# sqeazy/sqeazy

Hardware: AMD Instinct MI355X
Metric: encode GB/s (input voxels) for bitswap1->lz4 uint16 volume (higher is better)
Workload: dtype u16

## Files before the change

sqeazy_amd/csrc/sqy_kernels.hip:

```cpp
#include <hip/hip_runtime.h>
#include <atomic>
#include <mutex>
#include <stdint.h>
#include <cstring>
#include <type_traits>

#include "sqy_kernels.h"
#include "sqy_pipeline.hpp"
#include "sqy_quantiser_lut.hpp"
#include "sqy_batch_view.hpp"
#include "sqy_batch_window.hpp"

namespace sqy {

struct __attribute__((packed)) pk_u16 { uint16_t v; };
struct __attribute__((packed)) pk_u32 { uint32_t v; };
struct __attribute__((packed)) pk_u64 { uint64_t v; };
struct __attribute__((packed)) pk_u128 { uint32_t x, y, z, w; };

__device__ __forceinline__ uint32_t ld_u32(const uint8_t* p) { return reinterpret_cast<const pk_u32*>(p)->v; }
__device__ __forceinline__ uint64_t ld_u64(const uint8_t* p) { return reinterpret_cast<const pk_u64*>(p)->v; }
__device__ __forceinline__ uint4 ld_u128(const uint8_t* p)
{
    const pk_u128 t = *reinterpret_cast<const pk_u128*>(p);
// ... 633 lines not shown
    {
        const uint16_t* prev = out + (uint64_t)(z0 - 1u) * frame;
#pragma unroll
        for (uint32_t k = 0; k < DDK_ITEMS; ++k) {
            if (!it_on[k]) continue;
            uint16_t* d = img[0] + (size_t)it_i[k] * pitch + 8u;
            if (it_v[k] < vpr) *reinterpret_cast<uint4*>(d + it_v[k] * 8u) = *reinterpret_cast<const uint4*>(prev + (uint64_t)it_y[k] * X + it_v[k] * 8u);
            else d[w] = w < X ? prev[(uint64_t)it_y[k] * X + w] : (uint16_t)0;
        }
    }
    uint4 cin[DDK_ITEMS];
#pragma unroll
    for (uint32_t k = 0; k < DDK_ITEMS; ++k) cin[k] = active(k, 0) ? fetch(k, 0) : make_uint4(0, 0, 0, 0);
    __syncthreads();
    int cur = 0;
    for (uint32_t j = 0; j < nframes; ++j) {
        const uint32_t z = z0 + j;
        uint4 nin[DDK_ITEMS];
#pragma unroll
        for (uint32_t k = 0; k < DDK_ITEMS; ++k) nin[k] = (j + 1u < nframes && active(k, j + 1u)) ? fetch(k, j + 1u) : make_uint4(0, 0, 0, 0);
        uint16_t* dst = out + (uint64_t)z * frame;
        const uint16_t* A = img[cur];
        uint16_t* B = img[cur ^ 1];
        const bool frame_touched = z >= 1u && z < zlim && hx > 0u;
#pragma unroll
        for (uint32_t k = 0; k < DDK_ITEMS; ++k) {
            if (!active(k, j)) continue;
            const uint32_t i = it_i[k], v = it_v[k];
            const int32_t y = it_y[k];
            if (v == vpr) {
                B[(size_t)i * pitch + 8u + w] = (uint16_t)cin[k].x;
                continue;
            }
            const uint32_t x0 = v * 8u;
            const uint4 c = cin[k];
            uint32_t val[8] = {c.x & 0xffffu, c.x >> 16, c.y & 0xffffu, c.y >> 16, c.z & 0xffffu, c.z >> 16, c.w & 0xffffu, c.w >> 16};
            if (frame_touched && y >= 1 && y + 2 <= (int32_t)Y && x0 < 1u + hx) {
                uint32_t colsum[10];
#pragma unroll
                for (int q = 0; q < 10; ++q) colsum[q] = 0;
#pragma unroll
                for (int dy = -1; dy <= 1; ++dy) {
                    const uint16_t* r = A + (size_t)((int32_t)i + dy) * pitch + 8u + x0;
                    const uint4 e = *reinterpret_cast<const uint4*>(r);
                    colsum[0] += r[-1];
                    colsum[1] += e.x & 0xffffu; colsum[2] += e.x >> 16; colsum[3] += e.y & 0xffffu; colsum[4] += e.y >> 16;
                    colsum[5] += e.z & 0xffffu; colsum[6] += e.z >> 16; colsum[7] += e.w & 0xffffu; colsum[8] += e.w >> 16;
                    colsum[9] += r[8];
                }
#pragma unroll
                for (int q = 0; q < 8; ++q) {
                    const uint32_t x = x0 + (uint32_t)q;
                    if (x >= 1u && x < 1u + hx) {
                        const uint32_t sum = (colsum[q] + colsum[q + 1] + colsum[q + 2]) & 0xffffu;
                        val[q] = (val[q] + ((sum * 58255u) >> 19)) & 0xffffu;
                    }
                }
            }
            const uint4 o = make_uint4(val[0] | (val[1] << 16), val[2] | (val[3] << 16), val[4] | (val[5] << 16), val[6] | (val[7] << 16));
            *reinterpret_cast<uint4*>(B + (size_t)i * pitch + 8u + x0) = o;
            if (y >= y0 && y < y0 + (int32_t)DDK_R) *reinterpret_cast<uint4*>(dst + (uint64_t)y * X + x0) = o;
        }
        __syncthreads();
        cur ^= 1;
#pragma unroll
        for (uint32_t k = 0; k < DDK_ITEMS; ++k) cin[k] = nin[k];
    }
}

__global__ __launch_bounds__(DDK_THREADS)
void diff3x3x1_u16_decode_frames_kernel(const uint16_t* __restrict__ in, uint16_t* __restrict__ out, uint32_t Y, uint32_t X, uint32_t hx,
                                        uint32_t zlim, uint32_t w, uint32_t z0, uint32_t nframes)
{
    diff3x3x1_u16_decode_strip(in, out, Y, X, hx, zlim, w, z0, nframes, (int32_t)(blockIdx.x * DDK_R));
}

__device__ __forceinline__ uint32_t batch_job_of(const uint32_t* __restrict__ first, uint32_t njobs, uint32_t block)
{
    uint32_t lo = 0, hi = njobs;
    while (hi - lo > 1u) {
        const uint32_t mid = (lo + hi) >> 1;
        if (first[mid] <= block) lo = mid; else hi = mid;
    }
    return lo;
}

__global__ __launch_bounds__(256)
void diff3x3x1_decode_batch_copy_kernel(const DiffBatchJob* __restrict__ jobs, const uint32_t* __restrict__ first_tile, uint32_t njobs)
{
    const uint32_t j = batch_job_of(first_tile, njobs, blockIdx.x);
    const DiffBatchJob job = jobs[j];
    const uint32_t tile = blockIdx.x - first_tile[j];
    const uint32_t vpr = job.X / 8u, wv = job.w / 8u, zlim = job.X < job.Z ? job.X : job.Z;
    const uint64_t fv = (uint64_t)job.Y * vpr, nvec = (uint64_t)job.Z * fv;
    const uint4* __restrict__ in = static_cast<const uint4*>(job.in);
    uint4* __restrict__ out = static_cast<uint4*>(job.out);
#pragma unroll 4
    for (uint32_t i = 0; i < BSWB_THREAD_VOX / 8u; ++i) {
        const uint64_t v = (uint64_t)tile * (BSWB_TILE_VOX / 8u) + i * 256u + threadIdx.x;
        if (v >= nvec) break;
        const uint32_t z = (uint32_t)(v / fv), xv = (uint32_t)((v - (uint64_t)z * fv) % vpr);
        if (z >= 1u && z < zlim && xv < wv) continue;
        out[v] = in[v];
    }
}

__global__ __launch_bounds__(DDK_THREADS)
void diff3x3x1_decode_batch_kernel(const DiffBatchJob* __restrict__ jobs, const uint32_t* __restrict__ first_strip, uint32_t njobs, uint32_t step)
{
    const uint32_t j = batch_job_of(first_strip, njobs, blockIdx.x);
    const DiffBatchJob job = jobs[j];
    const uint32_t strip = blockIdx.x - first_strip[j];
    const uint32_t zlim = job.X < job.Z ? job.X : job.Z, z0 = 1u + step * DDK_K;
    if (z0 >= zlim) return;
    const uint32_t nframes = zlim - z0 < DDK_K ? zlim - z0 : DDK_K;
    diff3x3x1_u16_decode_strip(static_cast<const uint16_t*>(job.in), static_cast<uint16_t*>(job.out), job.Y, job.X, job.Z - 2u, zlim, job.w, z0, nframes,
                               (int32_t)(strip * DDK_R));
}

constexpr uint32_t LZ4_MFLIMIT = 12, LZ4_LASTLITERALS = 5, LZ4_MINLENGTH = 13, LZ4_MAXD = 65535;

__device__ __forceinline__ uint32_t lz4_hash5(uint64_t seq)
{
    return (uint32_t)(((seq << 24) * 889523592379ULL) >> 52);
}

__device__ __forceinline__ uint32_t lz4_hash5_32(uint32_t lo, uint32_t byte4)
{
    const uint32_t plo = 0x1BBCDCBBu;
    const uint32_t l = lo * plo;
    uint32_t h = __umulhi(lo, plo);
    h += (lo & 0xffu) * 0xCFu + (byte4 & 0xffu) * 0xBBu;
    return ((h << 4) | (l >> 28)) & 0xfffu;
}

#ifdef SQY_EXP_STATS
__device__ unsigned long long* g_exp_buf;
__device__ unsigned long long g_exp_cap;
extern "C" __attribute__((visibility("default"))) int SQYAMD_Exp_Set_Buffer(void* p, unsigned long long cap_records)
{
    unsigned long long* q = static_cast<unsigned long long*>(p);
    if (hipMemcpyToSymbol(HIP_SYMBOL(g_exp_buf), &q, sizeof q) != hipSuccess) return 1;
    return hipMemcpyToSymbol(HIP_SYMBOL(g_exp_cap), &cap_records, sizeof cap_records) != hipSuccess;
}
#define SQY_EXP(...) __VA_ARGS__
#else
#define SQY_EXP(...)
#endif
constexpr uint32_t LZ4_RINGLESS_U = 64u * 15u;
#ifndef SQY_EXP_WIN_LEAN
#define SQY_EXP_WIN_LEAN 8192
#endif
#ifndef SQY_EXP_DG_AHEAD
#define SQY_EXP_DG_AHEAD 8
#endif
constexpr uint32_t LZ4_WIN_LEAN = SQY_EXP_WIN_LEAN, LZ4_WIN_DENSE = 32768, LZ4_FB = 1024, LZ4_AHEAD = 2048, LZ4_MIRROR = 16;

template <uint32_t LZ4_WIN>
struct Lz4WindowT {
    glb_u8* src;
    lds_u8* win;
    uint32_t n;
    uint32_t whi, wlo;
    uint32_t nif;
    uint32_t lane16;
    uint32_t pmin;
    SQY_EXP(unsigned long long x_wait = 0; uint32_t x_nwait = 0;)

    __device__ __forceinline__ void issue()
    {
        const uint32_t b = whi + nif * LZ4_FB;
        if (b + LZ4_FB - wlo > LZ4_WIN) wlo = b + LZ4_FB - LZ4_WIN;
        const uint32_t a = b + lane16;
        if (a + 16u <= n) {
            const uint32_t lds_dst = (uint32_t)(uintptr_t)win + (b & (LZ4_WIN - 1));
            uint32_t keep;
            asm volatile("s_mov_b32 %0, m0\n\ts_mov_b32 m0, %2\n\ts_nop 0\n\tglobal_load_lds_dwordx4 %1, off\n\ts_mov_b32 m0, %0"
                         : "=&s"(keep) : "v"(src + a), "s"(lds_dst) : "memory");
        }
        nif += 1;
    }
    __device__ __forceinline__ void commit()
    {
        SQY_EXP(const unsigned long long x_t0 = __builtin_amdgcn_s_memtime();)
        asm volatile("s_waitcnt vmcnt(0)" ::: "memory");
        SQY_EXP(x_wait += __builtin_amdgcn_s_memtime() - x_t0; x_nwait += 1;)
        wave_lds_sync();
        const uint32_t end = whi + nif * LZ4_FB;
        if (((end - 1u) & ~(LZ4_WIN - 1)) != ((whi - 1u) & ~(LZ4_WIN - 1)) || whi == 0) {
            if (lane16 < 64u) *reinterpret_cast<SQY_LDS uint32_t*>(win + LZ4_WIN + (lane16 >> 2)) = *reinterpret_cast<const SQY_LDS uint32_t*>(win + (lane16 >> 2));
            wave_lds_sync();
        }
        whi = end;
        nif = 0;
    }
    __device__ __forceinline__ void ensure(uint32_t ip)
    {
        if (ip + LZ4_AHEAD <= whi || whi >= n) return;
        if (ip >= whi + (LZ4_WIN - LZ4_FB)) {
            asm volatile("s_waitcnt vmcnt(0)" ::: "memory");
            uint32_t start = ip & ~(LZ4_FB - 1);
            if (start >= pmin + LZ4_FB) start -= LZ4_FB;
            whi = wlo = start;
            nif = 0;
        }
        while (whi + nif * LZ4_FB < ip + LZ4_AHEAD && whi + nif * LZ4_FB < n) issue();
        commit();
        if (whi < n) issue();
    }
    __device__ __forceinline__ uint32_t hi_valid() const { return whi < (n & ~15u) ? whi : (n & ~15u); }
    __device__ __forceinline__ bool inside(uint32_t p, uint32_t len) const { return p >= wlo && p + len <= hi_valid(); }
    __device__ __forceinline__ const lds_u8* at(uint32_t p) const { return win + (p & (LZ4_WIN - 1)); }

    __device__ __forceinline__ uint4 lds128(uint32_t p) const { return lds_ld_u128(at(p)); }
    __device__ __forceinline__ uint32_t lds32(uint32_t p) const { return lds_ld_u32(at(p)); }
    __device__ __forceinline__ uint32_t lds8(uint32_t p) const { return lds_ld_u8(at(p)); }

    __device__ __forceinline__ uint64_t rd64(uint32_t p) const
    {
        uint64_t v;
        if (inside(p, 8)) v = lds_ld_u64(at(p)); else v = glb_ld_u64(src + p);
        return v;
    }
    __device__ __forceinline__ uint32_t rd32(uint32_t p) const
    {
        uint32_t v;
        if (inside(p, 4)) v = lds_ld_u32(at(p)); else v = glb_ld_u32(src + p);
        return v;
    }
    __device__ __forceinline__ uint32_t rd8(uint32_t p) const
    {
        uint32_t v;
        if (inside(p, 1)) v = lds_ld_u8(at(p)); else v = glb_ld_u8(src + p);
        return v;
    }
    __device__ __forceinline__ uint4 rd128(uint32_t p) const
    {
        uint4 v;
        if (inside(p, 16)) v = lds_ld_u128(at(p)); else v = glb_ld_u128(src + p);
        return v;
    }
};

template <class Lz4Window>
__device__ __forceinline__ void wave_copy(uint8_t* __restrict__ d, const Lz4Window& w, uint32_t from, uint32_t len, int lane)
{
    if (len <= 64) {
        if ((uint32_t)lane < len) d[lane] = (uint8_t)w.rd8(from + lane);
        return;
    }
    const uint32_t head = (uint32_t)((16 - (reinterpret_cast<uintptr_t>(d) & 15)) & 15);
    if ((uint32_t)lane < head) d[lane] = (uint8_t)w.rd8(from + lane);
    d += head; from += head; len -= head;
    const uint32_t nvec = len >> 4;
    for (uint32_t i = lane; i < nvec; i += 64) {
        *reinterpret_cast<uint4*>(d + (size_t)i * 16) = w.rd128(from + i * 16);
    }
    const uint32_t done = nvec << 4;
    if ((uint32_t)lane < len - done) d[done + lane] = (uint8_t)w.rd8(from + done + lane);
}

__device__ __forceinline__ uint32_t ffbl(uint32_t v)
{
    uint32_t r;
    asm("v_ffbl_b32 %0, %1" : "=v"(r) : "v"(v));
    return r;
}
__device__ __forceinline__ uint32_t first_nonzero16(uint32_t x0, uint32_t x1, uint32_t x2, uint32_t x3)
{
    const uint32_t t0 = ffbl(x0);
    const uint32_t t1 = ffbl(x1) | 32u;
    const uint32_t t2 = ffbl(x2) | 64u;
    const uint32_t t3 = ffbl(x3) | 96u;
    const uint32_t a = t0 < t1 ? t0 : t1, b = t2 < t3 ? t2 : t3;
    const uint32_t m = a < b ? a : b;
    return (m < 128u ? m : 128u) >> 3;
}
__device__ __forceinline__ uint32_t first_diff16(uint4 x, uint4 y)
{
    const uint32_t t0 = ffbl(x.x ^ y.x);
    const uint32_t t1 = ffbl(x.y ^ y.y) | 32u;
    const uint32_t t2 = ffbl(x.z ^ y.z) | 64u;
    const uint32_t t3 = ffbl(x.w ^ y.w) | 96u;
    const uint32_t a = t0 < t1 ? t0 : t1, b = t2 < t3 ? t2 : t3;
    const uint32_t m = a < b ? a : b;
    return (m < 128u ? m : 128u) >> 3;
}

template <class Lz4Window>
__device__ __forceinline__ uint32_t common16(const Lz4Window& w, uint32_t a, uint32_t b, uint32_t maxlen)
{
    if (a + 16u <= w.n) {
        const uint32_t c = first_diff16(w.rd128(a), w.rd128(b));
        return c < maxlen ? c : maxlen;
    }
    uint32_t c = 0;
    while (c < maxlen && glb_ld_u8(w.src + a + c) == glb_ld_u8(w.src + b + c)) ++c;
    return c;
}

constexpr uint32_t LZ4_OB = 2048;

struct Lz4Out {
    SQY_GLB uint8_t* dst;
    lds_u8* ob;
    uint32_t base;
    int lane;
// ... 93 lines not shown
                    za = (qa.x | qa.y | qa.z | qa.w) == 0u;
                    zb = (qb.x | qb.y | qb.z | qb.w) == 0u;
                }
            }
            x[u] = za ? zero : (v4u)a[pc * 64u + lane];
            y[u] = zb ? zero : (v4u)b[pc * 64u + lane];
        }
        uint32_t d = 0;
#pragma unroll
        for (uint32_t u = 0; u < 4; ++u) d |= (x[u].x ^ y[u].x) | (x[u].y ^ y[u].y) | (x[u].z ^ y[u].z) | (x[u].w ^ y[u].w);
        diff = ballot(d != 0u) != 0ull ? 1u : 0u;
    }
    if (lane == 0) dd.dup_of[k] = diff ? (uint32_t)k : r;
    return diff == 0u;
}

template <bool LINKED> struct Lz4ExtraArgs { typedef Lz4DedupeArgs type; };
template <> struct Lz4ExtraArgs<true> { typedef Lz4SpecArgs type; };
__device__ __forceinline__ uint32_t lz4_linked_tag_shift(uint32_t max_block)
{
    const uint32_t pmax = LZ4_HIST + max_block;
    return 31u - (32u - (uint32_t)__builtin_clz(pmax - 1));
}

template <bool LINKED, bool DENSE, bool ACCEL = false, bool TABLE = false>
__global__ __launch_bounds__(64)
void lz4_chunks_kernel(const uint8_t* __restrict__ in, uint64_t total, uint32_t chunk, uint64_t in_stride,
                       uint8_t* __restrict__ scratch, uint64_t stride, uint32_t* __restrict__ csize,
                       const uint64_t* __restrict__ fmap, uint64_t fbytes,
                       const Lz4Block* __restrict__ blocks, const uint32_t* __restrict__ frame_first, uint32_t max_block,
                       uint32_t* __restrict__ redo_list, const uint32_t* __restrict__ dup_of, uint32_t accel, typename Lz4ExtraArgs<LINKED>::type dd SQY_DIAG_ARG)
{
#ifdef SQY_LZ4_DIAG
    unsigned long long dacc = 0, dt0 = 0, dcnt = 0, dreason[16] = {0};
    bool darmed = false;
#endif
    __shared__ uint32_t table[4096];
    constexpr uint32_t LZ4_WIN = DENSE ? LZ4_WIN_DENSE : LZ4_WIN_LEAN;
    typedef Lz4WindowT<LZ4_WIN> Lz4Window;
    __shared__ __attribute__((aligned(16))) uint8_t ring[LZ4_WIN + LZ4_MIRROR];
    __shared__ __attribute__((aligned(16))) uint8_t stage[LZ4_OB];
    const int lane = threadIdx.x;
    if (!LINKED && !DENSE && dup_of && dup_of[blockIdx.x] != blockIdx.x) return;
    if constexpr (!LINKED && !DENSE && !ACCEL && !TABLE) if (dd.chunk_key) {
        if (lz4_chunk_dedupe(in, chunk, in_stride, total, blockIdx.x, dd, threadIdx.x)) return;
        asm volatile("s_waitcnt vmcnt(0)" ::: "memory");
    }
    SQY_EXP(const unsigned long long x_start = __builtin_amdgcn_s_memrealtime(); const unsigned long long x_c0 = __builtin_amdgcn_s_memtime();
            unsigned long long x_far = 0, x_commit = 0; uint32_t x_nfar = 0, x_ncommit = 0, x_nseq = 0, x_ngen = 0;
            unsigned long long x_acc[8] = {0, 0, 0, 0, 0, 0, 0, 0}; unsigned long long x_last = x_c0;
            auto x_lap = [&](int i) { const unsigned long long t = __builtin_amdgcn_s_memtime(); x_acc[i] += t - x_last; x_last = t; };)
    uint32_t b_first, b_last;
    uint32_t b_out = 0;
    uint32_t spec_mode = 0;
    if constexpr (LINKED) {
        spec_mode = dd.mode;
        if (spec_mode) {
            b_first = dd.wave_first[blockIdx.x];
            b_last = dd.wave_last[blockIdx.x] + 1u;
            b_out = spec_mode == 1u ? b_last - 1u : b_first;
        } else {
            b_first = frame_first[blockIdx.x];
            b_last = frame_first[blockIdx.x + 1];
            b_out = b_first;
        }
    } else {
        b_first = DENSE ? redo_list[1 + blockIdx.x] : blockIdx.x;
        b_last = b_first + 1;
    }
    uint32_t n_prev = 0;
  for (uint32_t bi = b_first; bi < b_last; ++bi) {
    const uint64_t blk = LINKED && bi < b_out ? b_last - 1u : bi;
    const uint32_t p0 = LINKED ? LZ4_HIST : 0u;
    uint32_t n, p_lo = 0;
    int64_t low_in = 0, low_dict = 0;
    bool fresh = true;
    const uint8_t* __restrict__ src;
    uint64_t tab_slot = 0;
    if (LINKED) {
        const Lz4Block bd = blocks[bi];
        n = bd.n;
        src = in + bd.start - LZ4_HIST;
        p_lo = bd.start >= LZ4_HIST ? 0u : (uint32_t)(LZ4_HIST - bd.start);
        low_in = bd.low_in - (int64_t)bd.start + LZ4_HIST;
        low_dict = bd.low_dict - (int64_t)bd.start + LZ4_HIST;
        fresh = (bd.flags & 1u) != 0;
        if constexpr (LINKED) {
            if (spec_mode == 1u && bi == b_first) fresh = true;
            if (spec_mode == 2u && bi == b_first && !fresh) {
                const uint32_t* __restrict__ tf = dd.tables + (uint64_t)(bi - 1u) * kLz4SpecTableWords + 4096u;
#pragma unroll 4
                for (int i = 0; i < 64; ++i) table[i * 64 + lane] = tf[i * 64 + lane];
                n_prev = blocks[bi - 1u].n;
            }
        }
    } else {
        if constexpr (TABLE) {
            const Lz4BatchChunk e = reinterpret_cast<const Lz4BatchChunk*>(blocks)[blk];
            src = in + e.off;
            n = e.n;
            tab_slot = e.slot;
        } else {
        const uint64_t lin = blk * chunk;
        src = fmap ? in + fmap[lin / fbytes] * fbytes + lin % fbytes : in + blk * in_stride;
        const uint64_t left = total - blk * chunk;
        n = (uint32_t)(left < chunk ? left : chunk);
        }
    }
    const uint32_t pend = p0 + n;
    auto back_room = [&](uint32_t mt) -> uint32_t {
        if (!LINKED) return mt;
        const int64_t r = (int64_t)mt - (mt >= p0 ? low_in : low_dict);
        return r < 0 ? 0u : (r > 0x7fffffff ? 0x7fffffffu : (uint32_t)r);
    };
    uint8_t* __restrict__ dst = scratch + (TABLE ? tab_slot : blk) * stride;

    Lz4Window w;
    w.src = (glb_u8*)src; w.win = (lds_u8*)ring; w.n = pend; w.whi = p0; w.wlo = p0; w.nif = 0; w.lane16 = (uint32_t)lane * 16u;
    w.pmin = p0;
    w.issue();
    Lz4Out o;
    o.dst = (SQY_GLB uint8_t*)dst; o.ob = (lds_u8*)stage; o.base = 0; o.lane = lane;
    const uint32_t pmax = LINKED ? LZ4_HIST + max_block : n;
    const uint32_t pos_bits = pmax > 1 ? 32u - (uint32_t)__builtin_clz(pmax - 1) : 1u;
    const uint32_t tsh = 31u - pos_bits;
    const uint32_t tmask = (1u << tsh) - 1u;
    auto tag_of = [&](uint32_t seq32) -> uint32_t { return (seq32 * 2654435761u) >> (32u - tsh); };
    if (fresh) {
        const uint32_t e0 = (p0 << tsh) | (n >= 4 ? tag_of(glb_ld_u32((glb_u8*)src + p0)) : 0u);
        uint4* t4 = reinterpret_cast<uint4*>(table);
#pragma unroll
        for (int i = 0; i < 16; ++i) t4[i * 64 + lane] = make_uint4(e0, e0, e0, e0);
        if constexpr (LINKED) if (spec_mode && bi >= b_out && !(blocks[bi].flags & 1u)) {
            uint4* g4 = reinterpret_cast<uint4*>(dd.tables + (uint64_t)bi * kLz4SpecTableWords);
#pragma unroll
            for (int i = 0; i < 16; ++i) g4[i * 64 + lane] = make_uint4(e0, e0, e0, e0);
        }
    } else {
#pragma unroll 4
        for (int i = 0; i < 64; ++i) {
            const uint32_t e = table[i * 64 + lane];
            const uint32_t pp = e >> tsh;
            const uint32_t e2 = pp >= n_prev ? (((pp - n_prev) << tsh) | (e & tmask)) : 0u;
            table[i * 64 + lane] = e2;
            if constexpr (LINKED) if (spec_mode && bi >= b_out) dd.tables[(uint64_t)bi * kLz4SpecTableWords + i * 64 + lane] = e2;
        }
    }
    __syncthreads();
    n_prev = n;

    const uint32_t* __restrict__ dgp = nullptr;
    uint32_t dg_words = 0;
    constexpr int DG_AHEAD = SQY_EXP_DG_AHEAD;
    uint32_t dgq[DG_AHEAD];
    uint32_t dgq_U = 0xffffffffu;
#pragma unroll
    for (int k = 0; k < DG_AHEAD; ++k) dgq[k] = 0u;
    if constexpr (!LINKED && !DENSE && !ACCEL && !TABLE) {
        if (dd.digest && n == chunk && dd.holes_map &&
            (uint32_t)dd.holes_map[blk * (1u + ((chunk >> 10) + 63u) / 64u)] == 0u) {
            dgp = dd.digest + blk * (uint64_t)dd.digest_stride;
            dg_words = dd.digest_stride;
        }
    }
    const uint32_t olimit = n - 1;
    uint32_t op = 0, anchor = p0;
    bool failed = false;
    bool redo_dense = false;

    if (n >= LZ4_MINLENGTH) {
        const uint32_t mflimitPlusOne = pend - LZ4_MFLIMIT + 1;
        const uint32_t matchlimit = pend - LZ4_LASTLITERALS;
        if (LINKED && !fresh) {
            const uint64_t s0 = glb_ld_u64((glb_u8*)src + p0);
            if (lane == 0) table[lz4_hash5(s0)] = (p0 << tsh) | tag_of((uint32_t)s0);
            wave_lds_sync();
        }
        uint32_t P = p0 + 1, U = 1;
        uint32_t put2 = 0xffffffffu;

        bool dense_next = DENSE;
        uint32_t shorts = 0;
        bool pend = false;
        uint32_t pe_lit = 0, pe_mcode = 0, pe_off = 0;
        uint32_t pe_litv = 0;
        uint32_t pe_bytes = 0, pe_ext = 0;
        auto emit_pending_checks = [&]() {
            const uint32_t lit = pe_lit, matchCode = pe_mcode;
            pe_ext = (matchCode + 240u) / 255u;
            pe_bytes = 1u + lit + 2u + pe_ext;
            if (op + 33u > olimit &&
                (op + 1u + lit + (2 + 1 + LZ4_LASTLITERALS) > olimit ||
                 op + 1u + lit + 2u + (1 + LZ4_LASTLITERALS) + pe_ext > olimit)) { failed = true; return; }
            o.reserve(op, pe_bytes);
        };
        auto emit_pending_bytes = [&]() {
            pend = false;
            const uint32_t lit = pe_lit, matchCode = pe_mcode, ml_ext = pe_ext;
            const uint32_t rest = matchCode - 15u - (ml_ext - 1u) * 255u;
            const uint64_t ones = (1ull << (8u * (ml_ext ? ml_ext - 1u : 0u))) - 1ull;
            const uint64_t tail = (uint64_t)pe_off | (ml_ext ? ((ones | ((uint64_t)rest << (8u * (ml_ext - 1u)))) << 16) : 0ull);
            const uint32_t k = (uint32_t)lane;
            const uint32_t j = k - (lit + 1u);
            const uint32_t tb = (uint32_t)(tail >> (8u * (j & 7u))) & 0xffu;
            uint32_t v = (lit << 4) | (matchCode < 15u ? matchCode : 15u);
            v = (k - 1u) < lit ? pe_litv : v;
            v = k > lit ? tb : v;
            if (k < pe_bytes) *o.at(op + k) = (uint8_t)v;
            op += pe_bytes;
        };
        auto emit_pending = [&]() {
            emit_pending_checks();
            if (failed) { pend = false; return; }
            emit_pending_bytes();
        };

        for (;;) {
            SQY_STAMP(0);
            SQY_EXP(x_lap(0);)
            if (ACCEL || U < LZ4_RINGLESS_U) w.ensure(P);

            uint32_t f = 64, fcand = 0;
            uint32_t ipf = 0;
            uint32_t fwl = 0;
            bool fw_exact = false;
            uint32_t bkl = 0xffffffffu;
            bool batch_done = false;
            uint32_t nvalid = 64, next_P = 0;

            bool finished = false;
            bool redo = false;
            if (DENSE && U == 0 && dense_next) {
                for (;;) {
                    if (!(P >= w.wlo + 4u && P + 112u <= w.hi_valid() && P + 112u <= matchlimit)) { dense_next = false; break; }
                    SQY_STAMP(20);
                    if (pend) { emit_pending(); if (failed) break; }
                    const uint32_t pos = P + (uint32_t)lane;
                    const uint32_t wlo4 = w.wlo + 4u;
                    const uint4 s16 = w.lds128(pos);
                    const uint32_t b4 = w.lds32(pos - 4u);
                    {
                        const uint32_t lo2 = (b4 >> 16) | (s16.x << 16);
                        const uint32_t h2 = lz4_hash5_32(lo2, s16.x >> 16);
                        if (lane == 0) atomicMax(&table[h2], ((P - 2u) << tsh) | tag_of(lo2));
                        wave_lds_sync();
                        put2 = 0xffffffffu;
                    }
                    const uint32_t h = lz4_hash5_32(s16.x, s16.y);
                    const uint32_t mytag = tag_of(s16.x);
                    const uint32_t mine = (pos << tsh) | mytag;
                    const uint32_t oe = table[h];
                    atomicMax(&table[h], 0x80000000u | (uint32_t)(63 - lane));
                    const uint32_t fl = table[h];
                    table[h] = oe;
                    wave_lds_sync();
                    const bool dup = (63u - (fl & 63u)) != (uint32_t)lane;
                    const uint32_t old = oe >> tsh;
                    const bool near = (pos - old) <= LZ4_MAXD && (oe & tmask) == mytag;
                    const bool cin = near && old >= wlo4;
                    uint4 c16 = w.lds128(old);
                    uint32_t cb4 = w.lds32(old - 4u);
                    if (ballot(near && !cin)) {
                        if (near && !cin) {
                            c16 = glb_ld_u128(w.src + old);
                            cb4 = old >= p_lo + 4u ? glb_ld_u32(w.src + old - 4u) : (glb_ld_u32(w.src + p_lo) << (8u * (4u - (old - p_lo))));
                        }
                    }
                    const uint32_t d = first_diff16(s16, c16);
                    const uint32_t xb = b4 ^ cb4;
                    const uint32_t bkv = xb ? ((uint32_t)__builtin_clz(xb) >> 3) : 4u;
                    auto verdict_word = [&](uint32_t fwd, uint32_t bk, uint32_t cand, uint32_t off) -> uint32_t {
                        const bool edge = cand < p_lo + 16u || (LINKED && back_room(cand) < 4u);
                        const uint32_t ml1 = (fwd == 16u || edge) ? 0u : (bk == 4u ? 5u : 15u);
                        return fwd | (bk << 5) | (ml1 << 8) | (fwd >= 4u ? 1u << 12 : 0u) | (off << 16);
                    };
                    const uint32_t info = (verdict_word(d, bkv, old, pos - old) & (near ? ~0u : ~(1u << 12))) | (dup ? 1u << 13 : 0u);
                    const uint64_t M = ballot(near && d >= 4u);
                    const uint64_t D = ballot(dup);
                    SQY_STAMP(21);
                    uint32_t cur = 0;
                    uint64_t chain = 0;
                    bool keep_dense = true;
                    uint64_t evm = M | D;
                    constexpr uint32_t W_OK = 0u, W_NONE = 1u, W_LIMIT = 2u, W_MATE = 3u;
                    uint32_t epk, einf;
                    {
                        const uint64_t x = evm >> (uint32_t)lane;
                        const uint32_t eo = x ? (uint32_t)__builtin_ctzll(x) : 0u;
                        const uint32_t e = (uint32_t)lane + eo;
                        einf = (uint32_t)__builtin_amdgcn_ds_bpermute((int)(e << 2), (int)info);
                        const uint32_t st = !x ? W_NONE : ((einf >> 13) & 1u) ? W_MATE : (eo >= ((einf >> 8) & 15u)) ? W_LIMIT : W_OK;
                        epk = st | (e << 8) | ((e + (einf & 31u)) << 16);
                    }
                    auto entered = [&](uint32_t q) -> bool {
                        if (q >= cur) return true;
                        const uint64_t cs = chain & ((2ull << q) - 1ull);
                        const uint32_t c = 63u - (uint32_t)__builtin_clzll(cs);
                        const uint32_t wq = lane_read(epk, c);
                        const uint32_t fqc = (wq >> 8) & 63u, nxc = wq >> 16;
                        return q <= fqc || q + 2u == nxc;
                    };
                    for (;;) {
                        uint32_t st, t0;
                        SQY_STAMP(24);
                        asm volatile(
                            "1:\n\t"
// ... 102 lines not shown
                        const uint32_t keep = (1u << hs) - 1u;
#pragma unroll
                        for (uint32_t i = 0; i < 6u; ++i)
                            wv[i] = i < hw ? wv[i] : (i == hw ? ((wv[i] & keep) | (uint32_t)hdr) : (i == hw + 1u ? (uint32_t)(hdr >> 32) : 0u));
                        lds_u8* const my = o.at(my_op);
#pragma unroll
                        for (uint32_t i = 0; i < 4u; ++i)
                            if (4u * (i + 1u) <= sb) reinterpret_cast<SQY_LDS pk_u32*>(my + 4u * i)->v = wv[i];
                        {
                            const uint32_t tw = sb >> 2, tb = sb & 3u;
                            const uint32_t tv = tw == 0 ? wv[0] : tw == 1 ? wv[1] : tw == 2 ? wv[2] : tw == 3 ? wv[3] : wv[4];
                            if (tb >= 1u) my[4u * tw] = (uint8_t)tv;
                            if (tb >= 2u) my[4u * tw + 1u] = (uint8_t)(tv >> 8);
                            if (tb >= 3u) my[4u * tw + 2u] = (uint8_t)(tv >> 16);
                        }
                        op += total;
                    }
                    anchor = P + cur;
                    put2 = anchor - 2u;
                    P = anchor;
                    SQY_STAMP(23);
                    w.ensure(P);
                    if (!keep_dense) { dense_next = false; break; }
                }
                if (failed) break;
            }
            if (!ACCEL && U == 0) {
                __builtin_amdgcn_s_waitcnt(0x0F70);
                const bool putlane = lane == 15;
                const uint32_t posoff = putlane ? 0xfffffffeu : (uint32_t)lane;
                const uint32_t notprobe = (uint32_t)lane < 15u ? 0u : 1u;
                const uint32_t lane0_off = lane == 0 ? 0u : 0xffffffffu;
                for (;;) {
                    {
                        const uint32_t hv = sgpr(w.hi_valid());
                        const uint32_t top = hv < matchlimit ? hv : matchlimit;
                        if (!(P >= sgpr(w.wlo) + 4u && P + 1200u <= top)) break;
                    }
                    SQY_STAMP(1);
                    const uint32_t pos = P + posoff;
                    const uint32_t wlo8 = w.wlo + 8u;
                    const uint32_t sh1 = pos & 3u;
                    const uint4 d1 = lds_ld_4dw(w.win + ((pos - 4u - sh1) & (LZ4_WIN - 1u)));
                    const uint32_t b4 = __builtin_amdgcn_alignbyte(d1.y, d1.x, sh1);
                    const uint2 s16 = make_uint2(__builtin_amdgcn_alignbyte(d1.z, d1.y, sh1), __builtin_amdgcn_alignbyte(d1.w, d1.z, sh1));
                    if (pend) { emit_pending_checks(); if (failed) break; }
                    SQY_STAMP(2);
                    const uint32_t h = lz4_hash5_32(s16.x, s16.y);
                    const uint32_t mytag = tag_of(s16.x);
                    const uint32_t mine = (pos << tsh) | mytag;
                    if (putlane) table[h] = mine;
                    wave_lds_sync();
                    put2 = 0xffffffffu;
                    SQY_STAMP(3);
                    const uint32_t oe = table[h];
                    if (pend) emit_pending_bytes();
                    const uint32_t old = oe >> tsh;
                    const uint32_t rej = ((oe & tmask) ^ mytag) | ((pos - old) >> 16) | notprobe;
                    SQY_STAMP(4);
                    const uint64_t nm = ballot(rej == 0u);
                    if (nm == 0) { SQY_REASON(0); break; }
                    const uint32_t f0 = ctz64(nm);
                    const uint32_t mt0 = lane_read(old, f0);
                    const uint32_t ip0 = P + f0;
                    if (mt0 < p_lo + 8u) { SQY_REASON(3); break; }
                    SQY_STAMP(5);
                    const bool commit = (uint32_t)lane <= f0;
                    if (commit) table[h] = mine;
                    wave_lds_sync();
                    const uint32_t rb = table[h];
                    const uint32_t r3 = ip0 & 3u;
                    const uint32_t hd = 4u + r3;
                    const uint32_t dd = (uint32_t)lane * 16u - hd;
                    uint32_t x0, x1, x2, x3;
                    if (mt0 >= wlo8) {
                        uint32_t oi = (ip0 + dd) & (LZ4_WIN - 1u), om = (mt0 + dd) & (LZ4_WIN - 1u);
                        asm volatile("" : "+v"(oi), "+v"(om));
                        const uint4 ci = lds_ld_4dw(w.win + oi), cm = lds_ld_u128(w.win + om);
                        x0 = ci.x ^ cm.x; x1 = ci.y ^ cm.y; x2 = ci.z ^ cm.z; x3 = ci.w ^ cm.w;
                    } else {
                        SQY_EXP(const unsigned long long x_t0 = __builtin_amdgcn_s_memtime();)
                        const uint4 cg = glb_ld_u128(w.src + (uint32_t)(mt0 + dd));
                        SQY_EXP(asm volatile("s_waitcnt vmcnt(0)" ::: "memory"); x_far += __builtin_amdgcn_s_memtime() - x_t0; x_nfar += 1;)
                        const uint4 ci = lds_ld_4dw(w.win + ((ip0 + dd) & (LZ4_WIN - 1u)));
                        x0 = ci.x ^ cg.x; x1 = ci.y ^ cg.y; x2 = ci.z ^ cg.z; x3 = ci.w ^ cg.w;
                        asm volatile("" : "+v"(x0));
                        SQY_REASON(2);
                    }
                    const uint32_t xbv = __builtin_amdgcn_alignbyte(x1, x0, r3);
                    x0 &= lane0_off;
                    x1 &= lane0_off | (0xffffffffu << (8u * r3));
                    const uint32_t g = first_nonzero16(x0, x1, x2, x3);
                    SQY_STAMP(6);
                    const uint64_t nf = ballot(g != 16u);
                    uint32_t eq = 1024u - hd;
                    bool settled = false;
                    if (nf) {
                        const uint32_t l = ctz64(nf);
                        eq = l * 16u + lane_read(g, l) - hd;
                        settled = true;
                    }
                    SQY_STAMP(7);
                    if ((ballot(rb != mine) & ((2ull << f0) - 1ull)) != 0ull || eq < 4u) {
                        if (eq < 4u) SQY_REASON(1); else SQY_REASON(3);
                        if (commit) table[h] = oe;
                        wave_lds_sync();
                        break;
                    }
                    const uint32_t ml = eq - 4u;
                    const uint32_t xb = lane_read(xbv, 0);
                    const uint32_t bk = xb ? ((uint32_t)__builtin_clz(xb) >> 3) : 4u;
                    const uint32_t room0 = back_room(mt0);
                    const uint32_t lim = f0 < room0 ? f0 : room0;
                    const uint32_t bck = bk < lim ? bk : lim;
                    const bool slow_back = bk == 4u && lim > 4u;
                    SQY_STAMP(8);
                    if (!settled || slow_back) {
                        if (!settled) SQY_REASON(4); else SQY_REASON(5);
                        f = f0; fcand = mt0; ipf = ip0; fwl = ml; fw_exact = settled;
                        bkl = slow_back ? 0xffffffffu : bck;
                        batch_done = true;
                        break;
                    }
                    SQY_EXP(x_nseq += 1;)
                    pend = true; pe_lit = f0 - bck; pe_mcode = ml + bck; pe_off = ip0 - mt0;
                    pe_litv = b4 >> 24;
                    const uint32_t ipn = ip0 + 4u + ml;
                    anchor = ipn;
                    if (ipn >= mflimitPlusOne) { finished = true; break; }
                    put2 = ipn - 2u;
                    P = ipn;
                    SQY_STAMP(9);
                    w.ensure(P);
                    if (DENSE) {
                        shorts = ml < 12u ? shorts + 1u : 0u;
                        if (shorts >= 2u) { shorts = 0; dense_next = true; redo = true; break; }
                    } else if (!LINKED) {
                        shorts = ml < 12u ? shorts + 1u : (shorts > 4u ? shorts - 4u : 0u);
                        if (shorts >= 128u && redo_list) { redo_dense = true; break; }
                    } else if (LINKED) {
                        if constexpr (LINKED) if (spec_mode == 1u) {
                            shorts = ml < 12u ? shorts + 1u : (shorts > 4u ? shorts - 4u : 0u);
                            if (shorts >= 2048u && !(blocks[b_last - 1u].flags & 1u)) { redo_dense = true; break; }
                        }
                    }
                }
                SQY_EXP(x_lap(1);)
                if (finished || failed || redo_dense) break;
                if (redo) continue;
            }

            if (pend) { emit_pending(); if (failed) break; }
            while (!DENSE && !ACCEL && !batch_done && U >= LZ4_RINGLESS_U && put2 == 0xffffffffu) {
                auto geometry = [&](uint32_t& pos, uint32_t& nxt) -> bool {
                    const uint32_t s_first = (62 + U) >> 6;
                    const uint32_t ustar = 64 * (s_first + 1) - 62;
                    const uint32_t u = U + lane;
                    pos = P + s_first * lane + (u > ustar ? u - ustar : 0u);
                    nxt = pos + ((u >= ustar) ? s_first + 1 : s_first);
                    return ballot(nxt <= mflimitPlusOne) == ~0ull;
                };
                auto enter = [&](uint32_t h, uint32_t mytag, uint32_t pos, uint32_t nxt) -> bool {
                    const uint32_t mine = (pos << tsh) | mytag;
                    const uint32_t oe = table[h];
                    const uint32_t seen = atomicMax(&table[h], mine);
                    wave_lds_sync();
                    const bool hit_before = (oe & tmask) == mytag && (pos - (oe >> tsh)) <= LZ4_MAXD;
                    const uint32_t sp = seen >> tsh;
                    const bool in_batch = sp >= P && seen != oe;
                    const bool trouble = hit_before || (in_batch && (sp >= pos || (seen & tmask) == mytag));
                    if (ballot(trouble)) {
                        table[h] = oe;
                        wave_lds_sync();
                        return false;
                    }
                    P = lane_read(nxt, 63);
                    U += 64;
                    return true;
                };
                auto digest_ok = [&]() -> bool { return sgpr((uint32_t)(dgp && anchor == p0 && U >= 961u && U - 961u + 64u <= dg_words)) != 0u; };
                if (digest_ok()) {
                    SQY_GLB const uint32_t* const dg = (SQY_GLB const uint32_t*)dgp;
                    auto dg_fetch = [&](uint32_t ahead) -> uint32_t {
                        const uint32_t ix = U - 961u + 64u * ahead + (uint32_t)lane;
                        return dg[ix < dg_words ? ix : dg_words - 1u];
                    };
                    if (dgq_U != U) {
#pragma unroll
                        for (int k = 0; k < DG_AHEAD; ++k) dgq[k] = dg_fetch((uint32_t)k);
                    }
                    dgq_U = 0xffffffffu;
                    bool on = true;
#pragma unroll
                    for (int k = 0; k < DG_AHEAD; ++k) {
                        if (!on) continue;
                        uint32_t pos, nxt;
                        if (!digest_ok() || !geometry(pos, nxt)) { on = false; continue; }
                        const uint32_t e = dgq[k];
                        uint32_t h = e >> 17, mytag = e & 0x1ffffu;
                        if (ballot(e == 0xffffffffu)) {
                            if (e == 0xffffffffu) {
                                const uint64_t seq = glb_ld_u64(w.src + pos);
                                h = lz4_hash5(seq); mytag = tag_of((uint32_t)seq);
                            }
                        }
                        if (!enter(h, mytag, pos, nxt)) { on = false; continue; }
                        dgq[k] = dg_fetch((uint32_t)DG_AHEAD - 1u);
                    }
                    if (!on) break;
                    dgq_U = U;
                    continue;
                }
                uint32_t pos, nxt;
                if (!geometry(pos, nxt)) break;
                const uint64_t seq = glb_ld_u64(w.src + pos);
                if (!enter(lz4_hash5(seq), tag_of((uint32_t)seq), pos, nxt)) break;
            }
            SQY_EXP(x_lap(2);)
            SQY_EXP(x_ngen += 1;)
            if (!batch_done) {
                if (U != 0) SQY_REASON(6); else SQY_REASON(7);
                uint32_t pos, nxt;
                if (!ACCEL) {
                    const uint32_t s_first = (62 + U) >> 6 ? (62 + U) >> 6 : 1;
                    const uint32_t ustar = 64 * (s_first + 1) - 62;
                    const uint32_t u = U + lane;
                    const uint32_t bump = u > ustar ? u - ustar : 0;
                    pos = P + s_first * lane + bump;
                    const uint32_t adv = (u >= ustar) ? s_first + 1 : s_first;
                    nxt = pos + adv;
                } else {
                    auto S = [&](uint64_t u) -> uint64_t {
                        if (u <= 2) return u;
                        const uint64_t m = u - 2, q = m >> 6, r = m & 63;
                        return 2 + 64 * ((uint64_t)accel * q + q * (q - 1) / 2) + r * ((uint64_t)accel + q);
                    };
                    const uint64_t s0 = S(U), s1 = S((uint64_t)U + lane) - s0, s2 = S((uint64_t)U + lane + 1) - s0;
                    const uint64_t lim = (uint64_t)mflimitPlusOne + 1;
                    pos = (uint32_t)(P + s1 < lim ? P + s1 : lim);
                    nxt = (uint32_t)(P + s2 < lim ? P + s2 : lim);
                }
                const bool valid = nxt <= mflimitPlusOne;
                const uint64_t vmask = ballot(valid);
                nvalid = (uint32_t)__builtin_popcountll(vmask);

                uint64_t seq = 0;
                if (valid) seq = w.rd64(pos);
                if (put2 != 0xffffffffu) {
                    const uint64_t s2 = w.rd64(put2);
                    const uint32_t h2 = lz4_hash5(s2);
                    if (lane == 0) table[h2] = (put2 << tsh) | tag_of((uint32_t)s2);
                    wave_lds_sync();
                    put2 = 0xffffffffu;
                }
                uint32_t h = 0, oe = 0, fl = 0;
                if (valid) {
                    h = lz4_hash5(seq);
                    oe = table[h];
                    atomicMax(&table[h], 0x80000000u | (uint32_t)(63 - lane));
                    fl = table[h];
                }
                const uint32_t seq32 = (uint32_t)seq;
                const uint32_t mytag = tag_of(seq32);
                const uint32_t old = oe >> tsh;
                const bool hazard = valid && ((63u - (fl & 63u)) != (uint32_t)lane);
                const uint64_t hz = ballot(hazard);

                const bool near = valid && !hazard && (old + LZ4_MAXD >= pos) && (oe & tmask) == mytag;
                uint32_t m32 = ~seq32;
                if (near) m32 = w.rd32(old);
                const uint64_t mm = ballot(near && m32 == seq32);

                f = mm ? ctz64(mm) : 64u;
                if (f < 64) fcand = lane_read(old, f);

                uint64_t hzq = hz & ((f < 64) ? ((1ull << f) - 1ull) : ~0ull);
                while (hzq) {
                    const uint32_t c = ctz64(hzq);
                    hzq &= hzq - 1;
                    const uint32_t hc = lane_read(h, c);
                    const uint64_t grp = ballot(valid && h == hc) & ((1ull << c) - 1ull);
                    const uint32_t j = 63u - (uint32_t)__builtin_clzll(grp);
                    const uint32_t pj = lane_read(pos, j), pc = lane_read(pos, c);
                    if (pj + LZ4_MAXD >= pc && lane_read(seq32, j) == lane_read(seq32, c)) {
                        f = c;
                        fcand = pj;
                        break;
                    }
                }

                const uint32_t ncommit = (f < 64) ? f + 1 : nvalid;
                if (valid) table[h] = oe;
                if ((uint32_t)lane < ncommit) atomicMax(&table[h], (pos << tsh) | mytag);
                wave_lds_sync();
                if (f < 64) ipf = lane_read(pos, f);
                next_P = lane_read(nxt, 63);
                
            } else {
                next_P = P + 64u;
            }

            if (f >= 64) {
                if (nvalid < 64) break;
                P = sgpr(next_P);
                U += 64;
                SQY_EXP(x_lap(3);)
                continue;
            }

            SQY_EXP(x_lap(3);)
            const uint32_t ip0 = sgpr(ipf);
            const uint32_t mt0 = sgpr(fcand);
            fwl = sgpr(fwl);
            bkl = sgpr(bkl);
            const uint32_t q = ip0 + 4, r = mt0 + 4;

            uint32_t ml;
            if (fw_exact) {
                ml = fwl;
            } else {
                ml = fwl;
                auto settle = [&](const uint32_t (&got)[4], uint32_t T) -> bool {
#pragma unroll
                    for (uint32_t t = 0; t < 4; ++t) {
                        if (t < T) {
                            const uint64_t nf = ballot(got[t] != 16u);
                            if (nf) {
                                const uint32_t l = ctz64(nf);
                                ml += l * 16u + lane_read(got[t], l);
                                return true;
                            }
                            ml += 1024u;
                        }
                    }
                    return false;
                };
                const uint32_t src_end = matchlimit < (w.n & ~15u) ? matchlimit : (w.n & ~15u);
                for (;;) {
                    uint32_t got[4] = {0, 0, 0, 0};
                    const uint32_t qa = q + ml, ra = r + ml;
                    const uint32_t lds_end = w.hi_valid() < matchlimit ? w.hi_valid() : matchlimit;
                    if (ra >= w.wlo && qa + 1024u + 16u <= lds_end) {
                        uint32_t T = (lds_end - 16u - qa) >> 10;
                        T = T < 4u ? T : 4u;
                        got[0] = first_diff16(w.lds128(qa + (uint32_t)lane * 16u), w.lds128(ra + (uint32_t)lane * 16u));
                        if (T > 1u && !ballot(got[0] != 16u)) {
#pragma unroll
                            for (uint32_t t = 1; t < 4; ++t)
                                if (t < T) got[t] = first_diff16(w.lds128(qa + t * 1024u + (uint32_t)lane * 16u), w.lds128(ra + t * 1024u + (uint32_t)lane * 16u));
                        } else
                            T = 1;
                        if (settle(got, T)) break;
                        continue;
                    }
                    if (qa + 4096u + 16u <= src_end) {
                        uint4 ca[4], cb[4], na[4], nb[4];
                        auto load_round = [&](uint4 (&xa)[4], uint4 (&xb)[4], uint32_t ipos) {
#pragma unroll
                            for (uint32_t t = 0; t < 4; ++t) {
                                xa[t] = glb_ld_u128(w.src + ipos + t * 1024u + (uint32_t)lane * 16u);
// ... 6602 lines not shown
```

Baseline: 2125.

## Batch digest hash-table inserts in groups with one LDS sync per group

```diff
diff --git a/sqeazy_amd/csrc/sqy_kernels.hip b/sqeazy_amd/csrc/sqy_kernels.hip
--- a/sqeazy_amd/csrc/sqy_kernels.hip
+++ b/sqeazy_amd/csrc/sqy_kernels.hip
@@ -809,7 +809,10 @@
 #define SQY_EXP_WIN_LEAN 8192
 #endif
 #ifndef SQY_EXP_DG_AHEAD
-#define SQY_EXP_DG_AHEAD 8
+#define SQY_EXP_DG_AHEAD 16
+#endif
+#ifndef SQY_EXP_DG_GROUP
+#define SQY_EXP_DG_GROUP 16
 #endif
 constexpr uint32_t LZ4_WIN_LEAN = SQY_EXP_WIN_LEAN, LZ4_WIN_DENSE = 32768, LZ4_FB = 1024, LZ4_AHEAD = 2048, LZ4_MIRROR = 16;
 
@@ -1209,6 +1212,8 @@
     const uint32_t* __restrict__ dgp = nullptr;
     uint32_t dg_words = 0;
     constexpr int DG_AHEAD = SQY_EXP_DG_AHEAD;
+    constexpr int DG_GROUP = SQY_EXP_DG_GROUP;
+    static_assert(DG_AHEAD % DG_GROUP == 0, "a pass is a whole number of groups");
     uint32_t dgq[DG_AHEAD];
     uint32_t dgq_U = 0xffffffffu;
 #pragma unroll
@@ -1617,14 +1622,15 @@
 
             if (pend) { emit_pending(); if (failed) break; }
             while (!DENSE && !ACCEL && !batch_done && U >= LZ4_RINGLESS_U && put2 == 0xffffffffu) {
-                auto geometry = [&](uint32_t& pos, uint32_t& nxt) -> bool {
-                    const uint32_t s_first = (62 + U) >> 6;
+                auto geometry_at = [&](uint32_t Pk, uint32_t Uk, uint32_t& pos, uint32_t& nxt) -> bool {
+                    const uint32_t s_first = (62 + Uk) >> 6;
                     const uint32_t ustar = 64 * (s_first + 1) - 62;
-                    const uint32_t u = U + lane;
-                    pos = P + s_first * lane + (u > ustar ? u - ustar : 0u);
+                    const uint32_t u = Uk + lane;
+                    pos = Pk + s_first * lane + (u > ustar ? u - ustar : 0u);
                     nxt = pos + ((u >= ustar) ? s_first + 1 : s_first);
                     return ballot(nxt <= mflimitPlusOne) == ~0ull;
                 };
+                auto geometry = [&](uint32_t& pos, uint32_t& nxt) -> bool { return geometry_at(P, U, pos, nxt); };
                 auto enter = [&](uint32_t h, uint32_t mytag, uint32_t pos, uint32_t nxt) -> bool {
                     const uint32_t mine = (pos << tsh) | mytag;
                     const uint32_t oe = table[h];
@@ -1644,7 +1650,7 @@
                     return true;
                 };
                 auto digest_ok = [&]() -> bool { return sgpr((uint32_t)(dgp && anchor == p0 && U >= 961u && U - 961u + 64u <= dg_words)) != 0u; };
-                if (digest_ok()) {
+                if constexpr (!LINKED && !DENSE && !ACCEL && !TABLE) if (digest_ok()) {
                     SQY_GLB const uint32_t* const dg = (SQY_GLB const uint32_t*)dgp;
                     auto dg_fetch = [&](uint32_t ahead) -> uint32_t {
                         const uint32_t ix = U - 961u + 64u * ahead + (uint32_t)lane;
@@ -1657,20 +1663,81 @@
                     dgq_U = 0xffffffffu;
                     bool on = true;
 #pragma unroll
-                    for (int k = 0; k < DG_AHEAD; ++k) {
+                    for (int g = 0; g < DG_AHEAD / DG_GROUP; ++g) {
                         if (!on) continue;
-                        uint32_t pos, nxt;
-                        if (!digest_ok() || !geometry(pos, nxt)) { on = false; continue; }
-                        const uint32_t e = dgq[k];
-                        uint32_t h = e >> 17, mytag = e & 0x1ffffu;
-                        if (ballot(e == 0xffffffffu)) {
-                            if (e == 0xffffffffu) {
-                                const uint64_t seq = glb_ld_u64(w.src + pos);
-                                h = lz4_hash5(seq); mytag = tag_of((uint32_t)seq);
+                        uint32_t pos0, nxt0;
+                        geometry_at(P, U, pos0, nxt0);
+                        auto geometry_next = [&](uint32_t& Pj, uint32_t& pos, uint32_t& nxt) {
+                            const uint32_t dP = lane_read(nxt, 63) - Pj;
+                            Pj += dP; pos += dP + (uint32_t)lane; nxt += dP + (uint32_t)lane + 1u;
+                        };
+                        {
+                            bool own = false;
+#pragma unroll
+                            for (int j = 0; j < DG_GROUP; ++j) own = own || dgq[g * DG_GROUP + j] == 0xffffffffu;
+                            if (ballot(own)) {
+                                uint64_t seqj[DG_GROUP];
+                                uint32_t Pj = P, pos = pos0, nxt = nxt0;
+#pragma unroll
+                                for (int j = 0; j < DG_GROUP; ++j) {
+                                    seqj[j] = 0;
+                                    if (dgq[g * DG_GROUP + j] == 0xffffffffu && nxt <= mflimitPlusOne) seqj[j] = glb_ld_u64(w.src + pos);
+                                    geometry_next(Pj, pos, nxt);
+                                }
+#pragma unroll
+                                for (int j = 0; j < DG_GROUP; ++j)
+                                    if (dgq[g * DG_GROUP + j] == 0xffffffffu)
+                                        dgq[g * DG_GROUP + j] = (lz4_hash5(seqj[j]) << 17) | tag_of((uint32_t)seqj[j]);
                             }
                         }
-                        if (!enter(h, mytag, pos, nxt)) { on = false; continue; }
-                        dgq[k] = dg_fetch((uint32_t)DG_AHEAD - 1u);
+                        uint32_t nb = 0;
+                        uint32_t oe[DG_GROUP], seen[DG_GROUP];
+                        {
+                            uint32_t Pj = P, pos = pos0, nxt = nxt0;
+#pragma unroll
+                            for (int j = 0; j < DG_GROUP; ++j) {
+                                oe[j] = 0; seen[j] = 0;
+                                if (nb == (uint32_t)j && sgpr((uint32_t)(U + 64u * (uint32_t)j - 961u + 64u <= dg_words)) != 0u &&
+                                    lane_read(nxt, 63) <= mflimitPlusOne) {
+                                    nb = (uint32_t)j + 1u;
+                                    const uint32_t e = dgq[g * DG_GROUP + j];
+                                    const uint32_t h = e >> 17;
+                                    oe[j] = table[h];
+                                    seen[j] = atomicMax(&table[h], (pos << tsh) | (e & 0x1ffffu));
+                                }
+                                geometry_next(Pj, pos, nxt);
+                            }
+                        }
+                        wave_lds_sync();
+                        uint32_t bad = nb;
+                        uint32_t Pgood = P;
+                        {
+                            uint32_t Pj = P, pos = pos0, nxt = nxt0;
+#pragma unroll
+                            for (int j = 0; j < DG_GROUP; ++j) {
+                                if ((uint32_t)j < nb) {
+                                    const uint32_t mytag = dgq[g * DG_GROUP + j] & 0x1ffffu;
+                                    const bool hit_before = (oe[j] & tmask) == mytag && (pos - (oe[j] >> tsh)) <= LZ4_MAXD;
+                                    const uint32_t sp = seen[j] >> tsh;
+                                    const bool in_batch = sp >= Pj && seen[j] != oe[j];
+                                    const bool trouble = hit_before || (in_batch && (sp >= pos || (seen[j] & tmask) == mytag));
+                                    if (bad == nb && ballot(trouble)) bad = (uint32_t)j;
+                                }
+                                geometry_next(Pj, pos, nxt);
+                                if ((uint32_t)j < bad) Pgood = Pj;
+                            }
+                        }
+                        if (bad < nb) {
+#pragma unroll
+                            for (int j = DG_GROUP - 1; j >= 0; --j)
+                                if ((uint32_t)j < nb && (uint32_t)j >= bad) table[dgq[g * DG_GROUP + j] >> 17] = oe[j];
+                            wave_lds_sync();
+                        }
+                        P = Pgood;
+                        U += 64u * bad;
+                        if (bad < (uint32_t)DG_GROUP) { on = false; continue; }
+#pragma unroll
+                        for (int j = 0; j < DG_GROUP; ++j) dgq[g * DG_GROUP + j] = dg_fetch((uint32_t)(DG_AHEAD - DG_GROUP + j));
                     }
                     if (!on) break;
                     dgq_U = U;
```

New measurement: 2131, median of 3. About the same (+0.3%).
